# cvg/nice-slam

Hardware: NVIDIA H100
Metric: rendered rays/sec (higher is better)
Workload: dtype f32

## Files before the change

nice_slam_b200/csrc/nsb_aux.cu:

```cuda
#include <cstdarg>
#include <cstdio>
#include <cstring>
#include <cuda_fp16.h>
#include "nsb_common.cuh"
#include "nsb_seeds.cuh"
#include "nsb_geom.cuh"

namespace nsb {

static thread_local char g_err[512] = "";
void set_error(const char* fmt, ...) {
  va_list ap; va_start(ap, fmt); vsnprintf(g_err, sizeof(g_err), fmt, ap); va_end(ap);
}
int check_cuda(cudaError_t e, const char* what) {
  if (e == cudaSuccess) return NSB_OK;
  set_error("%s: %s", what, cudaGetErrorString(e));
  (void)cudaGetLastError();
  return NSB_ERR_CUDA;
}

struct PackArgs { nsb_decoder_params p[4]; float* packed[4]; float* flat[4]; int present[4]; };
__device__ __forceinline__ bool pk_mine(int& e) { return (e++ % (int)gridDim.y) == (int)blockIdx.y; }
constexpr int kPackSlices = 32;

// ... 175 lines not shown
  __shared__ float red[32];
  float m = -INFINITY;
  for (int i = threadIdx.x; i < n; i += blockDim.x) m = fmaxf(m, gt[i]);
  for (int o = 16; o > 0; o >>= 1) m = fmaxf(m, __shfl_xor_sync(0xffffffffu, m, o));
  if ((threadIdx.x & 31) == 0) red[threadIdx.x >> 5] = m;
  __syncthreads();
  if (threadIdx.x < 32) {
    m = threadIdx.x < (blockDim.x >> 5) ? red[threadIdx.x] : -INFINITY;
    for (int o = 16; o > 0; o >>= 1) m = fmaxf(m, __shfl_xor_sync(0xffffffffu, m, o));
    if (threadIdx.x == 0) {
      if (n <= 0) m = 0.0f;
      out2[0] = m;
      out2[1] = __fmul_rn(m, 1.2f);
    }
  }
  if (px.world > 1) {
    __shared__ uint32_t s_seq;
    __syncthreads();
    const uint32_t seq = peer_begin(px, 0, &s_seq);
    const int par = seq & 1u;
    if ((int)threadIdx.x < px.world) ll_put_f32(px.peer[threadIdx.x] + kXMaxOff + ((size_t)par * NSB_MAX_PEERS + px.rank) * 16, out2[0], seq);
    if (threadIdx.x < 32) {
      float mm = -INFINITY;
      if ((int)threadIdx.x < px.world) mm = ll_get_f32(px.peer[px.rank] + kXMaxOff + ((size_t)par * NSB_MAX_PEERS + threadIdx.x) * 16, seq, px, 0);
      for (int o = 16; o > 0; o >>= 1) mm = fmaxf(mm, __shfl_xor_sync(0xffffffffu, mm, o));
      if (threadIdx.x == 0) { out2[0] = mm; out2[1] = __fmul_rn(mm, 1.2f); }
    }
    peer_end(px, 0, seq);
  }
}

struct Bound6 { double b[6]; };
__global__ void prefilter_kernel(const float* __restrict__ ro, const float* __restrict__ rd, const float* __restrict__ gt,
                                 int n, const Bound6 B, uint8_t* __restrict__ keep) {
  const int i = blockIdx.x * blockDim.x + threadIdx.x;
  if (i >= n) return;
  const float o[3] = {ro[3 * i], ro[3 * i + 1], ro[3 * i + 2]}, d[3] = {rd[3 * i], rd[3 * i + 1], rd[3 * i + 2]};
  const double t = ray_far_bb(B.b, o, d);
  keep[i] = (t >= (double)gt[i]) ? 1 : 0;
}

__global__ void tracking_seeds_kernel(const double* __restrict__ depth, const double* __restrict__ var, const float* __restrict__ rgb,
                                      const float* __restrict__ gt, const double* __restrict__ gt_rgb, int n, double w_color,
                                      int handle_dynamic, int use_color, const double* __restrict__ pool, int n_pool,
                                      double* __restrict__ g_depth, float* __restrict__ g_rgb,
                                      double* __restrict__ loss, double* __restrict__ res, const PeerX px) {
  __shared__ __align__(16) unsigned char scratch[kSeedsScratchBytes];
// ... 720 lines not shown
```

nice_slam_b200/csrc/nsb_seeds.cuh:

```cuda
#pragma once
#include <cstdio>
#include "nsb_common.cuh"

namespace nsb {

constexpr long long kPeerWaitCycles = 20000000000ll;
constexpr size_t kXMaxOff = 0, kXSumOff = 256, kXSumStride = 256, kXPoolOff = kXSumOff + 2 * NSB_MAX_PEERS * kXSumStride;
__host__ __device__ inline size_t peer_pool_plain_off(int max_n) { return kXPoolOff + (size_t)2 * NSB_MAX_PEERS * (size_t)max_n * 16; }
__host__ __device__ inline size_t peer_buffer_bytes(int max_n) { return peer_pool_plain_off(max_n) + (size_t)NSB_MAX_PEERS * (size_t)max_n * sizeof(double); }
__device__ __forceinline__ void ll_put(unsigned char* slot16, double v, uint32_t seq) {
  const unsigned long long b = (unsigned long long)__double_as_longlong(v);
  const unsigned long long w0 = ((unsigned long long)seq << 32) | (b & 0xffffffffull), w1 = ((unsigned long long)seq << 32) | (b >> 32);
  asm volatile("st.relaxed.sys.global.v2.u64 [%0], {%1, %2};" ::"l"(slot16), "l"(w0), "l"(w1) : "memory");
}
__device__ __forceinline__ double ll_get(const unsigned char* slot16, uint32_t seq, const PeerX& px, int c) {
  unsigned long long w0, w1;
  const long long t0 = clock64();
  for (;;) {
    asm volatile("ld.relaxed.sys.global.v2.u64 {%0, %1}, [%2];" : "=l"(w0), "=l"(w1) : "l"(slot16) : "memory");
    if ((uint32_t)(w0 >> 32) == seq && (uint32_t)(w1 >> 32) == seq) break;
    if (clock64() - t0 > kPeerWaitCycles) { printf("nsb: peer exchange timed out (rank %d, channel %d, seq %u)\n", px.rank, c, seq); __trap(); }
  }
  return __longlong_as_double((long long)((w1 << 32) | (w0 & 0xffffffffull)));
}
__device__ __forceinline__ void ll_put_f32(unsigned char* slot8, float v, uint32_t seq) {
  const unsigned long long w = ((unsigned long long)seq << 32) | (unsigned long long)__float_as_uint(v);
  asm volatile("st.relaxed.sys.global.u64 [%0], %1;" ::"l"(slot8), "l"(w) : "memory");
}
__device__ __forceinline__ float ll_get_f32(const unsigned char* slot8, uint32_t seq, const PeerX& px, int c) {
  unsigned long long w;
  const long long t0 = clock64();
  for (;;) {
    asm volatile("ld.relaxed.sys.global.u64 %0, [%1];" : "=l"(w) : "l"(slot8) : "memory");
    if ((uint32_t)(w >> 32) == seq) break;
    if (clock64() - t0 > kPeerWaitCycles) { printf("nsb: peer exchange timed out (rank %d, channel %d, seq %u)\n", px.rank, c, seq); __trap(); }
  }
  return __uint_as_float((uint32_t)w);
}
__device__ __forceinline__ void peer_end(const PeerX& px, int c, uint32_t seq) {
  __syncthreads();
  if (threadIdx.x == 0) px.counter[c] = (unsigned long long)seq;
}
__device__ __forceinline__ uint32_t peer_begin(const PeerX& px, int c, uint32_t* s_seq) {
  if (threadIdx.x == 0) *s_seq = (uint32_t)(px.counter[c] + 1ull);
  __syncthreads();
  return *s_seq;
}

__device__ __forceinline__ float peer_max_all_ctas(const PeerX& px, float local, uint32_t* s_seq) {
  if (threadIdx.x == 0) *s_seq = (uint32_t)(px.counter[0] + 1ull);
  __syncthreads();
  const uint32_t seq = *s_seq;
  const int par = seq & 1u;
  __syncthreads();
  if (blockIdx.x == 0 && (int)threadIdx.x < px.world)
    ll_put_f32(px.peer[threadIdx.x] + kXMaxOff + ((size_t)par * NSB_MAX_PEERS + px.rank) * 16, local, seq);
  float m = -INFINITY;
  if (threadIdx.x < 32) {
    if ((int)threadIdx.x < px.world) m = ll_get_f32(px.peer[px.rank] + kXMaxOff + ((size_t)par * NSB_MAX_PEERS + threadIdx.x) * 16, seq, px, 0);
    for (int o = 16; o > 0; o >>= 1) m = fmaxf(m, __shfl_xor_sync(0xffffffffu, m, o));
    if (threadIdx.x == 0) *reinterpret_cast<float*>(s_seq) = m;
  }
  __syncthreads();
  m = *reinterpret_cast<const float*>(s_seq);
  __syncthreads();
  return m;
}
__device__ __forceinline__ void peer_advance(const PeerX& px, int c) {
  px.counter[c] = px.counter[c] + 1ull;
}
__device__ __forceinline__ void peer_sum13(const PeerX& px, const double* tot, int n_val, double* out, uint32_t* s_seq) {
  const uint32_t seq = peer_begin(px, 2, s_seq);
  const int par = seq & 1u;
  for (int i = threadIdx.x; i < n_val * px.world; i += blockDim.x) {
    const int r = i / n_val, k = i - n_val * r;
    ll_put(px.peer[r] + kXSumOff + ((size_t)par * NSB_MAX_PEERS + px.rank) * kXSumStride + (size_t)k * 16, tot[k], seq);
  }
  if ((int)threadIdx.x < n_val) {
    double v = 0.0;
    for (int r = 0; r < px.world; r++) v += ll_get(px.peer[px.rank] + kXSumOff + ((size_t)par * NSB_MAX_PEERS + r) * kXSumStride + (size_t)threadIdx.x * 16, seq, px, 2);
    out[threadIdx.x] = v;
  }
  peer_end(px, 2, seq);
}

constexpr int kMedianDirect = 512;
constexpr int kSeedsScratchBytes = 34 * 8 + kMedianDirect * 8 + (256 + 8 + 2 + 2) * 4;

__device__ __forceinline__ double block_sum(double v, double* red) {
  for (int o = 16; o > 0; o >>= 1) v += __shfl_xor_sync(0xffffffffu, v, o);
  if ((threadIdx.x & 31) == 0) red[threadIdx.x >> 5] = v;
  __syncthreads();
  double t = 0.0;
  if (threadIdx.x < 32) {
    t = threadIdx.x < (blockDim.x >> 5) ? red[threadIdx.x] : 0.0;
    for (int o = 16; o > 0; o >>= 1) t += __shfl_xor_sync(0xffffffffu, t, o);
  }
  __syncthreads();
  return t;
}
__device__ __forceinline__ double sgn(double x) { return (x > 0.0) - (x < 0.0); }

__device__ __forceinline__ void tracking_seeds_body(const double* depth, const double* var, const float* rgb,
// ... 6 lines not shown
  unsigned long long& med_key = *reinterpret_cast<unsigned long long*>(red + 33);
  unsigned long long* keys = reinterpret_cast<unsigned long long*>(red + 34);
  int* hist = reinterpret_cast<int*>(keys + kMedianDirect);
  int* wtot = hist + 256;
  int* sel = wtot + 8;
  uint32_t* s_seq_p = reinterpret_cast<uint32_t*>(sel + 2);
  for (int i = threadIdx.x; i < n; i += blockDim.x)
    res[i] = fabs((double)gt[i] - depth[i]) / sqrt(var[i] + 1e-10);
  __syncthreads();
  if (handle_dynamic) {
    const double* mp = pool != nullptr ? pool : res;
    int np = pool != nullptr ? n_pool : n;
    int pool_pitch = 0;
    if (px.world > 1) {
      const uint32_t seq = peer_begin(px, 1, s_seq_p);
      const int par = seq & 1u;
      for (int i = threadIdx.x; i < n * px.world; i += blockDim.x) {
        const int r = i / n, j = i - r * n;
        ll_put(px.peer[r] + kXPoolOff + (((size_t)par * NSB_MAX_PEERS + px.rank) * px.max_n + j) * 16, res[j], seq);
      }
      double* plain = reinterpret_cast<double*>(px.peer[px.rank] + peer_pool_plain_off(px.max_n));
      for (int i = threadIdx.x; i < n * px.world; i += blockDim.x) {
        const int r = i / n, j = i - r * n;
        plain[(size_t)r * px.max_n + j] = ll_get(px.peer[px.rank] + kXPoolOff + (((size_t)par * NSB_MAX_PEERS + r) * px.max_n + j) * 16, seq, px, 1);
      }
      peer_end(px, 1, seq);
      mp = plain;
      np = n * px.world; pool_pitch = px.max_n;
    }
    auto pool_at = [&](int i) { return pool_pitch ? mp[(size_t)(i / n) * pool_pitch + (i % n)] : mp[i]; };
    const int k = (np - 1) / 2;
    auto select_direct = [&](int cnt, int want) {
      if (cnt > 256) {
        int m = 512;
        for (int i = cnt + threadIdx.x; i < m; i += blockDim.x) keys[i] = ~0ull;
        __syncthreads();
        for (int k2 = 2; k2 <= m; k2 <<= 1)
          for (int j = k2 >> 1; j > 0; j >>= 1) {
            for (int t = threadIdx.x; t < m / 2; t += blockDim.x) {
              const int i = ((t & ~(j - 1)) << 1) | (t & (j - 1));
              const unsigned long long x = keys[i], y = keys[i | j];
              if ((x > y) == ((i & k2) == 0)) { keys[i] = y; keys[i | j] = x; }
            }
            __syncthreads();
          }
        if (threadIdx.x == 0) med_key = keys[want];
        __syncthreads();
// ... 123 lines not shown
```

nice_slam_b200/csrc/nsb_tc.cuh:

```cuda
#pragma once

namespace nsb {
namespace tc {

#ifdef NSB_PHASE_TIMING
__device__ long long g_phase[64];
__device__ long long g_phase_last;
#define NSB_PH(id) do { if (blockIdx.x == 0 && threadIdx.x == 0) { const long long c_ = clock64(); ::nsb::tc::g_phase[id] += c_ - ::nsb::tc::g_phase_last; ::nsb::tc::g_phase_last = c_; } } while (0)
#define NSB_PH_RESET() do { if (blockIdx.x == 0 && threadIdx.x == 0) ::nsb::tc::g_phase_last = clock64(); } while (0)
#else
#define NSB_PH(id) do { } while (0)
#define NSB_PH_RESET() do { } while (0)
#endif

constexpr int TM = 128;
constexpr int kThreads = 512;
constexpr int kCG = kThreads / TM;
constexpr int kCW = 32 / kCG;
constexpr int kKQ = kCW / 4;

__device__ __forceinline__ float to_tf32(float x) { return __uint_as_float(__float_as_uint(x) & 0xffffe000u); }

__device__ __forceinline__ int canon_q(int r, int kq, int K) { return ((r >> 3) * (K >> 2) + kq) * 32 + (r & 7) * 4; }

// ... 3 lines not shown
  h.x = to_tf32(v.x); h.y = to_tf32(v.y); h.z = to_tf32(v.z); h.w = to_tf32(v.w);
  l.x = v.x - h.x; l.y = v.y - h.y; l.z = v.z - h.z; l.w = v.w - h.w;
  *reinterpret_cast<float4*>(hi + idx) = h;
  *reinterpret_cast<float4*>(lo + idx) = l;
}

__device__ __forceinline__ uint64_t make_desc(const float* smem, uint32_t lbo_bytes, uint32_t sbo_bytes) {
  uint64_t d = 0;
  d |= (uint64_t)((smem_u32(smem) >> 4) & 0x3FFF);
  d |= (uint64_t)((lbo_bytes >> 4) & 0x3FFF) << 16;
  d |= (uint64_t)((sbo_bytes >> 4) & 0x3FFF) << 32;
  return d;
}

constexpr int kAccCols = 256;
constexpr int kAccSlotsPerSm = 4;
constexpr int kAccMaxSm = 144;
__device__ float g_acc_pool[(size_t)kAccMaxSm * kAccSlotsPerSm * kAccCols * TM];
__device__ int g_acc_lock[kAccMaxSm * kAccSlotsPerSm];
__shared__ float* s_acc;
__device__ __forceinline__ uint32_t acc_acquire() {
  uint32_t smid;
  asm volatile("mov.u32 %0, %%smid;" : "=r"(smid));
  if (smid >= (uint32_t)kAccMaxSm) { printf("nsb: SM id %u beyond the accumulator pool\n", smid); __trap(); }
  const long long t0 = clock64();
  for (;;) {
    for (int k = 0; k < kAccSlotsPerSm; k++) {
      const int s = (int)smid * kAccSlotsPerSm + k;
      if (atomicCAS(&g_acc_lock[s], 0, 1) == 0) {
        __threadfence();
        s_acc = g_acc_pool + (size_t)s * kAccCols * TM;
        return (uint32_t)s;
      }
    }
    if (clock64() - t0 > 4000000000ll) { printf("nsb: no free accumulator slot on SM %u\n", smid); __trap(); }
  }
}
__device__ __forceinline__ void acc_release(uint32_t slot) { __threadfence(); atomicExch(&g_acc_lock[slot], 0); }
__device__ __forceinline__ const float* acc_col(uint32_t taddr) { return s_acc + (size_t)(taddr & 0xffffu) * TM + (taddr >> 16) + (threadIdx.x & 31); }

__device__ __forceinline__ void wg_fence() { asm volatile("wgmma.fence.sync.aligned;" ::: "memory"); }
__device__ __forceinline__ void wg_commit_wait() {
  asm volatile("wgmma.commit_group.sync.aligned;" ::: "memory");
  asm volatile("wgmma.wait_group.sync.aligned 0;" ::: "memory");
}
__device__ __forceinline__ void wg_commit() { asm volatile("wgmma.commit_group.sync.aligned;" ::: "memory"); }
__device__ __forceinline__ void wg_wait0() { asm volatile("wgmma.wait_group.sync.aligned 0;" ::: "memory"); }
__device__ __forceinline__ void fence_acc(float (&d)[16]) {
#pragma unroll
  for (int e = 0; e < 16; e++) asm volatile("" : "+f"(d[e])::"memory");
}
#define NSB_WG_D16 "+f"(d[0]), "+f"(d[1]), "+f"(d[2]), "+f"(d[3]), "+f"(d[4]), "+f"(d[5]), "+f"(d[6]), "+f"(d[7]), \
                   "+f"(d[8]), "+f"(d[9]), "+f"(d[10]), "+f"(d[11]), "+f"(d[12]), "+f"(d[13]), "+f"(d[14]), "+f"(d[15])
__device__ __forceinline__ void wgmma_tf32_n32(float (&d)[16], uint64_t da, uint64_t db) {
  asm volatile("{\n\t.reg .pred p;\n\tsetp.ne.b32 p, 1, 0;\n\t"
               "wgmma.mma_async.sync.aligned.m64n32k8.f32.tf32.tf32 "
               "{%0,%1,%2,%3,%4,%5,%6,%7,%8,%9,%10,%11,%12,%13,%14,%15}, %16, %17, p, 1, 1;\n\t}"
               : NSB_WG_D16 : "l"(da), "l"(db));
// ... 457 lines not shown
```

nice_slam_b200/csrc/nsb_tile.cuh:

```cuda
#pragma once

namespace nsb {
namespace tl {

using tc::TM;
constexpr int kThreads = 256;
constexpr int kEpiThreads = kThreads;
constexpr int kCG = 2, kCW = 16, kKQ = 4;
constexpr int kSlots = 4;
constexpr int kSlotFloatsFwd = 2560;
constexpr int kSlotFloatsBwd = 2048;
constexpr int kABufFloats = 2 * TM * 32;
constexpr int kMaxTileRays = 18;
constexpr int kMinSamples = 8;
constexpr long long kWaitCycles = 4000000000ll;

enum { B_FULL = 0, B_EMPTY = 4, B_HDR = 8, B_AREADY = 10, B_DONE = 12, kNumBars = 14 };

__device__ __forceinline__ bool mbar_try(uint64_t* bar, uint32_t parity) {
  uint32_t ok;
  asm volatile("{\n\t.reg .pred p;\n\tmbarrier.try_wait.parity.shared::cta.b64 p, [%1], %2;\n\tselp.b32 %0, 1, 0, p;\n\t}"
               : "=r"(ok) : "r"(smem_u32(bar)), "r"(parity) : "memory");
  return ok != 0;
}
__device__ __forceinline__ bool mbar_test(uint64_t* bar, uint32_t parity) {
  uint32_t ok;
  asm volatile("{\n\t.reg .pred p;\n\tmbarrier.test_wait.parity.shared::cta.b64 p, [%1], %2;\n\tselp.b32 %0, 1, 0, p;\n\t}"
               : "=r"(ok) : "r"(smem_u32(bar)), "r"(parity) : "memory");
  return ok != 0;
}
__device__ __forceinline__ void mbar_wait_b(uint64_t* bar, uint32_t parity) {
  if (mbar_try(bar, parity)) return;
  const long long t0 = clock64();
  while (!mbar_try(bar, parity)) {
    if (clock64() - t0 > kWaitCycles) { printf("nsb: mbarrier wait timed out (block %d thread %d bar %p parity %u)\n", blockIdx.x, threadIdx.x, (void*)bar, parity); __trap(); }
  }
}
__device__ __forceinline__ void mbar_arrive(uint64_t* bar) {
  asm volatile("mbarrier.arrive.shared::cta.b64 _, [%0];" ::"r"(smem_u32(bar)) : "memory");
}
__device__ __forceinline__ void epi_sync() { __syncthreads(); }

struct TileSmem {
  float* a[2];
  float* ring;
  int slot_floats;
  float* hdr;
  uint64_t* bars;
  uint32_t* tmem;
  unsigned char* extra;
};
__host__ __device__ constexpr size_t common_bytes(bool bwd) {
  return (2 * (size_t)kABufFloats + (size_t)kSlots * (bwd ? kSlotFloatsBwd : kSlotFloatsFwd) + 2 * kHdrFloats) * 4 + 128;
}
__device__ __forceinline__ void carve(unsigned char* base, TileSmem& t, bool bwd) {
  float* f = reinterpret_cast<float*>(base);
  t.a[0] = f; f += kABufFloats; t.a[1] = f; f += kABufFloats;
  t.slot_floats = bwd ? kSlotFloatsBwd : kSlotFloatsFwd;
// ... 46 lines not shown
}
__device__ __forceinline__ void loader_top_up(Loader& L, const TileSmem& t, uint32_t issued) {
  while (!loader_done(L) && L.loaded < issued + kSlots) {
    if (L.loaded >= kSlots) { const uint32_t prev = L.loaded - kSlots; if (!mbar_test(t.bars + B_EMPTY + (prev & (kSlots - 1)), (prev >> 2) & 1u)) return; }
    loader_issue(L, t);
  }
}
__device__ __forceinline__ void load_header(const KParams& P, const TileSmem& t, int lv, int hb) {
  uint64_t* bar = t.bars + B_HDR + hb;
  mbar_expect_tx(bar, kHdrFloats * 4u);
  tma_bulk_g2s(t.hdr + hb * kHdrFloats, P.in.packed[lv] + op_fwd_offset(lv), kHdrFloats * 4u, bar);
}

struct Issuer {
  Loader L;
  uint32_t issued;
  uint32_t g;
};
__device__ __forceinline__ void issuer_wait_operands(Issuer& I, const TileSmem& t, int b, uint32_t parity) {
  uint64_t* bar = t.bars + B_AREADY + b;
  const long long t0 = clock64();
  while (!mbar_test(bar, parity)) {
    if (threadIdx.x == 0) loader_top_up(I.L, t, I.issued);
    if (clock64() - t0 > kWaitCycles) { printf("nsb: issuer timed out waiting for operands (block %d)\n", blockIdx.x); __trap(); }
  }
}
__device__ __forceinline__ const float* issuer_unit(Issuer& I, const TileSmem& t, uint32_t k = 0) {
  if (threadIdx.x == 0) {
    loader_top_up(I.L, t, I.issued);
    while (I.L.loaded <= I.issued + k) loader_refill(I.L, t, I.issued);
  }
  const uint32_t u = I.issued + k;
  const int slot = u & (kSlots - 1);
  mbar_wait_b(t.bars + B_FULL + slot, (u >> 2) & 1u);
  return t.ring + slot * t.slot_floats;
}
__device__ __forceinline__ const float* issued_unit(const Issuer& I, const TileSmem& t, uint32_t k) { return t.ring + ((I.issued + k) & (kSlots - 1)) * t.slot_floats; }

__device__ __forceinline__ uint32_t cvt_h2(float lo_elem, float hi_elem) {
  uint32_t r;
  asm("cvt.rn.satfinite.f16x2.f32 %0, %1, %2;" : "=r"(r) : "f"(hi_elem), "f"(lo_elem));
  return r;
}
__device__ __forceinline__ void split_h2(float x, float y, uint32_t& h, uint32_t& l) {
  h = cvt_h2(x, y);
  const float2 f = __half22float2(*reinterpret_cast<const __half2*>(&h));
  l = cvt_h2(x - f.x, y - f.y);
}
__device__ __forceinline__ void put4_h(float* tile, int r, int kq, const float4 v) {
  unsigned char* hi = reinterpret_cast<unsigned char*>(tile) + (((r >> 3) * 4 + (kq >> 1)) * 128 + (r & 7) * 16 + (kq & 1) * 8);
  uint2 h, l;
  split_h2(v.x, v.y, h.x, l.x); split_h2(v.z, v.w, h.y, l.y);
  *reinterpret_cast<uint2*>(hi) = h;
  *reinterpret_cast<uint2*>(hi + TM * 32 * 2) = l;
}
__device__ __forceinline__ void put16_h(float* tile, int r, int cg, const float (&v)[kCW]) {
#pragma unroll
  for (int c = 0; c < 2; c++) {
    unsigned char* hi = reinterpret_cast<unsigned char*>(tile) + (((r >> 3) * 4 + 2 * cg + c) * 128 + (r & 7) * 16);
    uint4 h, l;
    split_h2(v[8 * c], v[8 * c + 1], h.x, l.x); split_h2(v[8 * c + 2], v[8 * c + 3], h.y, l.y);
    split_h2(v[8 * c + 4], v[8 * c + 5], h.z, l.z); split_h2(v[8 * c + 6], v[8 * c + 7], h.w, l.w);
    *reinterpret_cast<uint4*>(hi) = h;
    *reinterpret_cast<uint4*>(hi + TM * 32 * 2) = l;
  }
}
template <bool H16>
__device__ __forceinline__ void mma_rows(float (&d)[16], const float* a, int ka0, const float* b, int N, int KB, int c, int ksteps) {
  const uint32_t g = (threadIdx.x >> 7) & 1u;
  const int esz = H16 ? 2 : 4, kcm = H16 ? 8 : 4;
  const uint32_t sbo_a = (32u / kcm) * 128u, sbo_b = (uint32_t)(KB / kcm) * 128u;
  uint64_t ah = tc::make_desc(a + (ka0 / kcm) * 32, 128u, sbo_a), bh = tc::make_desc(b, 128u, sbo_b);
  ah += (uint64_t)((8u * sbo_a * g) >> 4);
  bh += (uint64_t)((4u * sbo_b * (uint32_t)c) >> 4);
  const uint64_t al = ah + (uint64_t)((TM * 32 * esz) >> 4), bl = bh + (uint64_t)((N * KB * esz) >> 4);
#pragma unroll 1
  for (int ks = 0; ks < ksteps; ks++) {
    const uint64_t o = 16u * (uint64_t)ks;
    if (H16) { tc::wgmma_f16_n32(d, al + o, bh + o); tc::wgmma_f16_n32(d, ah + o, bl + o); tc::wgmma_f16_n32(d, ah + o, bh + o); }
    else { tc::wgmma_tf32_n32(d, al + o, bh + o); tc::wgmma_tf32_n32(d, ah + o, bl + o); tc::wgmma_tf32_n32(d, ah + o, bh + o); }
  }
}
__device__ __forceinline__ void release_units(Issuer& I, const TileSmem& t, uint32_t count, uint64_t* done = nullptr) {
  if ((threadIdx.x & 127) == 0) {
    for (uint32_t k = 0; k < count; k++) mbar_arrive(t.bars + B_EMPTY + ((I.issued + k) & (kSlots - 1)));
    if (done != nullptr) mbar_arrive(done);
  }
  I.issued += count;
}
__device__ __forceinline__ void wg_bar_sync() {
  if (threadIdx.x >> 7) asm volatile("bar.sync 2, 128;" ::: "memory");
  else asm volatile("bar.sync 1, 128;" ::: "memory");
}
__device__ __forceinline__ void zero16(float (&d)[16]) {
#pragma unroll
  for (int e = 0; e < 16; e++) d[e] = 0.0f;
}
__device__ __forceinline__ void put2(float* hi, int r, int c, float a, float b) {
  float* hp = hi + tc::canon_q(r, c >> 2, 32) + (c & 3);
  const float h0 = tc::to_tf32(a), h1 = tc::to_tf32(b);
  *reinterpret_cast<float2*>(hp) = make_float2(h0, h1);
  *reinterpret_cast<float2*>(hp + TM * 32) = make_float2(a - h0, b - h1);
}

__device__ __forceinline__ void publish(const TileSmem& t, int b) {
  fence_proxy_async();
  __syncwarp();
  if ((threadIdx.x & 31) == 0) mbar_arrive(t.bars + B_AREADY + b);
}
__device__ __forceinline__ void wait_group(const TileSmem& t, uint32_t m) {
  mbar_wait_b(t.bars + B_DONE + (m & 1u), (m >> 1) & 1u);
}

struct GatherPass {
  float4 v[8];
  float w[8];
  int src_lane;
};
template <bool FAST>
// ... 72 lines not shown
__device__ __forceinline__ float4* d2_frag(int i) { return reinterpret_cast<float4*>(tc::s_acc + ((size_t)i * kThreads + threadIdx.x) * 16); }
__device__ __forceinline__ void ld_frag(const float4* p, float (&d)[16]) {
#pragma unroll
  for (int k = 0; k < 4; k++) { const float4 v = p[k]; d[4 * k] = v.x; d[4 * k + 1] = v.y; d[4 * k + 2] = v.z; d[4 * k + 3] = v.w; }
}
__device__ __forceinline__ void st_frag(float4* p, const float (&d)[16]) {
#pragma unroll
  for (int k = 0; k < 4; k++) p[k] = make_float4(d[4 * k], d[4 * k + 1], d[4 * k + 2], d[4 * k + 3]);
}
template <bool H16 = false>
__device__ __forceinline__ void issue_fc(Issuer& I, const TileSmem& t, int half) {
  constexpr int nu = H16 ? 2 : 4;
  const int b = I.g & 1;
  issuer_wait_operands(I, t, b, (I.g >> 1) & 1u);
#pragma unroll 1
  for (int u = 0; u < nu; u++) issuer_unit(I, t, u);
#pragma unroll 1
  for (int c = 0; c < 5; c++) {
    float4* p = d2_frag(c);
    float d[16];
    if (half == 0) zero16(d); else ld_frag(p, d);
    tc::wg_fence();
#pragma unroll
    for (int u = 0; u < nu; u++) mma_rows<H16>(d, t.a[b], H16 ? 16 * u : 8 * u, issued_unit(I, t, u), 160, H16 ? 16 : 8, c, 1);
    tc::wg_commit(); tc::wg_wait0(); tc::fence_acc(d);
    st_frag(p, d);
  }
  release_units(I, t, nu, t.bars + B_DONE + b);
  I.g++;
}
template <bool H16 = false>
__device__ __forceinline__ void issue_l0(Issuer& I, const TileSmem& t, float (&d1)[16], float (&d3)[16]) {
  constexpr int nu = H16 ? 1 : 2;
  const int b = I.g & 1;
  issuer_wait_operands(I, t, b, (I.g >> 1) & 1u);
#pragma unroll 1
  for (int u = 0; u < nu; u++) issuer_unit(I, t, u);
  tc::wg_fence();
#pragma unroll
  for (int u = 0; u < nu; u++) {
    mma_rows<H16>(d1, t.a[b], 16 * u, issued_unit(I, t, u), 64, H16 ? 32 : 16, 0, 2);
    mma_rows<H16>(d3, t.a[b], 16 * u, issued_unit(I, t, u), 64, H16 ? 32 : 16, 1, 2);
  }
  tc::wg_commit(); tc::wg_wait0(); tc::fence_acc(d1); tc::fence_acc(d3);
  release_units(I, t, nu, t.bars + B_DONE + b);
  I.g++;
}
template <bool H16 = false>
__device__ __forceinline__ void issue_h(Issuer& I, const TileSmem& t, float (&d1)[16], const float (&d3)[16], const float* hbuf, int i) {
  const float* w = issuer_unit(I, t);
  if (i == 3) {
#pragma unroll
    for (int e = 0; e < 16; e++) d1[e] = d3[e];
  } else {
    zero16(d1);
  }
  tc::wg_fence();
  mma_rows<H16>(d1, hbuf, 0, w, 32, 32, 0, H16 ? 2 : 4);
  tc::wg_commit();
}

template <bool H16 = false>
__device__ __forceinline__ void epi_forward(const KParams& P, const TileSmem& t, Issuer& I, int lv, const PointGeom& G, uint32_t& n, int hb, uint32_t hdr_parity,
                                            float (&out)[4], uint32_t* __restrict__ masks, float* __restrict__ acts, int npts) {
  const int row = threadIdx.x & (TM - 1), cg = threadIdx.x >> 7, warp = threadIdx.x >> 5, lane = threadIdx.x & 31;
  const bool xyz = lv != 0;
  const int cd = op_cd(lv), no = lv == 3 ? 4 : 1;
  const float* hdr = t.hdr + hb * kHdrFloats;
  float d1[16], d3[16];
  zero16(d1); zero16(d3);
  if (xyz) {
    for (int half = 0; half < cd / 32; half++) {
      if (n >= 2) wait_group(t, n - 2);
      if (threadIdx.x == 0) loader_top_up(I.L, t, I.issued);
      gather_tile<H16>(P.in.grid[half == 0 ? lv : 1], t.a[n & 1], G.xn, warp, lane);
      NSB_PH(1);
      publish(t, n & 1); n++;
      issue_fc<H16>(I, t, half);
      NSB_PH(2);
    }
    mbar_wait_b(t.bars + B_HDR + hb, hdr_parity);
    for (int blk = 0; blk < 3; blk++) {
      if (n >= 2) wait_group(t, n - 2);
      if (threadIdx.x == 0) loader_top_up(I.L, t, I.issued);
      NSB_PH(6);
      embed_tile<H16>(t.a[n & 1], hdr + 464, G.pf, row, cg, blk);
      NSB_PH(3);
      publish(t, n & 1); n++;
      issue_l0<H16>(I, t, d1, d3);
      NSB_PH(4);
    }
  } else {
    if (n >= 2) wait_group(t, n - 2);
    gather_tile<H16>(P.in.grid[0], t.a[n & 1], G.xnc, warp, lane);
    publish(t, n & 1); n++;
    issue_l0<H16>(I, t, d1, d3);
    mbar_wait_b(t.bars + B_HDR + hb, hdr_parity);
  }
  st_frag(d2_frag(5), d3);
  float* hbuf = t.a[n & 1];
  const int wg = threadIdx.x >> 7, q = lane & 3;
  const int r0 = 64 * wg + 16 * (warp & 3) + (lane >> 2);
#pragma unroll 1
  for (int i = 0; i < 5; i++) {
    float v2[16];
    if (xyz) ld_frag(d2_frag(i), v2);
    if (i > 0) { tc::wg_wait0(); tc::fence_acc(d1); release_units(I, t, 1); }
    if (threadIdx.x == 0) loader_top_up(I.L, t, I.issued);
    NSB_PH(7);
    uint32_t m0 = 0, m1 = 0;
#pragma unroll
    for (int e = 0; e < 16; e++) {
      const int c = 8 * (e >> 2) + 2 * q + (e & 1);
      const float u = d1[e] + hdr[i * 32 + c];
      const uint32_t bit = u > 0.0f ? 1u << (8 * (e >> 2) + (e & 1)) : 0u;
      if (e & 2) m1 |= bit; else m0 |= bit;
      float h = u > 0.0f ? u : 0.0f;
      if (xyz) h += v2[e] + hdr[160 + i * 32 + c];
      d1[e] = h;
    }
    if (masks != nullptr) {
      m0 <<= 2 * q; m1 <<= 2 * q;
      m0 |= __shfl_xor_sync(0xffffffffu, m0, 1); m1 |= __shfl_xor_sync(0xffffffffu, m1, 1);
      m0 |= __shfl_xor_sync(0xffffffffu, m0, 2); m1 |= __shfl_xor_sync(0xffffffffu, m1, 2);
      if (q == 0 && r0 < npts) masks[(size_t)r0 * 15 + i] = m0;
      if (q == 1 && r0 + 8 < npts) masks[(size_t)(r0 + 8) * 15 + i] = m1;
    }
    if (acts != nullptr) {
#pragma unroll
      for (int e = 0; e < 16; e += 2) {
// ... 1 lines not shown
        if (r < npts) __stcg(reinterpret_cast<float2*>(acts + (size_t)r * 160 + i * 32 + c), make_float2(d1[e], d1[e + 1]));
      }
    }
    if (i == 4) break;
    if (i == 2) ld_frag(d2_frag(5), d3);
#pragma unroll
    for (int e = 0; e < 16; e += 2) {
      const int r = r0 + 8 * ((e >> 1) & 1), c = 8 * (e >> 2) + 2 * q;
      if (H16) {
        unsigned char* hp = reinterpret_cast<unsigned char*>(hbuf) + (((r >> 3) * 4 + (c >> 3)) * 128 + (r & 7) * 16 + (c & 7) * 2);
        uint32_t hh, ll;
        split_h2(d1[e], d1[e + 1], hh, ll);
        *reinterpret_cast<uint32_t*>(hp) = hh;
        *reinterpret_cast<uint32_t*>(hp + TM * 32 * 2) = ll;
      } else {
        put2(hbuf, r, c, d1[e], d1[e + 1]);
      }
    }
    NSB_PH(8);
    fence_proxy_async();
    wg_bar_sync();
    issue_h<H16>(I, t, d1, d3, hbuf, i + 1);
    NSB_PH(9);
  }
  NSB_PH(8);
  float s0[4], s1[4];
#pragma unroll
  for (int o = 0; o < 4; o++) {
    s0[o] = s1[o] = 0.0f;
    if (o < no) {
#pragma unroll
      for (int e = 0; e < 16; e++) {
        const float w = hdr[336 + o * 32 + 8 * (e >> 2) + 2 * q + (e & 1)];
        if (e & 2) s1[o] = fmaf(d1[e], w, s1[o]); else s0[o] = fmaf(d1[e], w, s0[o]);
      }
    }
    s0[o] += __shfl_xor_sync(0xffffffffu, s0[o], 1); s1[o] += __shfl_xor_sync(0xffffffffu, s1[o], 1);
    s0[o] += __shfl_xor_sync(0xffffffffu, s0[o], 2); s1[o] += __shfl_xor_sync(0xffffffffu, s1[o], 2);
  }
  constexpr int kWgHiFloats = 64 * 32 / (H16 ? 2 : 1);
  auto part = [&](int r) { return reinterpret_cast<float4*>(hbuf + (r >> 6) * kWgHiFloats + (r & 63) * 4); };
  if (q == 0) *part(r0) = make_float4(s0[0], s0[1], s0[2], s0[3]);
  if (q == 1) *part(r0 + 8) = make_float4(s1[0], s1[1], s1[2], s1[3]);
  epi_sync();
  {
    const float4 v = *part(row);
// ... 32 lines not shown
__device__ __forceinline__ void gather_tile_kt(const nsb_grid& g, float* c_hi, int lo_off, const float xn[3], int warp, int lane) {
  const bool fast = grid_fast(g);
  const int qd = warp & 3, it0 = (warp >> 2) * 4, q = lane & 7;
#pragma unroll 1
  for (int it = it0; it < it0 + 4; it++) {
    GatherPass A;
    if (fast) gather_issue<true>(g, xn, it, lane, A); else gather_issue<false>(g, xn, it, lane, A);
    float4 acc = make_float4(0.f, 0.f, 0.f, 0.f);
#pragma unroll
    for (int k = 0; k < 8; k++) {
      const float w = A.w[k];
      acc.x = fmaf(A.v[k].x, w, acc.x); acc.y = fmaf(A.v[k].y, w, acc.y); acc.z = fmaf(A.v[k].z, w, acc.z); acc.w = fmaf(A.v[k].w, w, acc.w);
    }
    const int p = qd * 32 + A.src_lane;
    float4 xh, xl; split4(acc, xh, xl);
    const float hv[4] = {xh.x, xh.y, xh.z, xh.w}, lv[4] = {xl.x, xl.y, xl.z, xl.w};
#pragma unroll
    for (int c = 0; c < 4; c++) { const int o = kt_idx(4 * q + c, p); c_hi[o] = hv[c]; c_hi[lo_off + o] = lv[c]; }
  }
}
__device__ __forceinline__ void wg_group(WgSmem& w, int part, float* dst, int pitch, int n_rows, bool transposed3 = false) {
  fence_proxy_async();
  __syncthreads();
  if (threadIdx.x < 128) {
    const uint64_t ah = tc::make_desc(w.du, 128u, 4096u), al = ah + (uint64_t)((kWgALo * 4) >> 4);
    const uint64_t bh = tc::make_desc(w.b, 128u, 4096u), bl = bh + (uint64_t)((kWgBLo * 4) >> 4);
    float d[16];
#pragma unroll
    for (int e = 0; e < 16; e++) d[e] = 0.0f;
    tc::wg_fence();
#pragma unroll 1
    for (int ks = 0; ks < TM / 8; ks++) {
      const uint64_t o = 16u * (uint64_t)ks;
      tc::wgmma_tf32_n32(d, al + o, bh + o); tc::wgmma_tf32_n32(d, ah + o, bl + o); tc::wgmma_tf32_n32(d, ah + o, bh + o);
    }
    tc::wg_commit_wait();
    if ((threadIdx.x >> 6) == part) {
#pragma unroll
      for (int e = 0; e < 16; e += 2) {
        int r, c; tc::frag_rc(e, r, c); r -= 32 * part;
        if (r >= n_rows) continue;
        if (transposed3) {
          if (c < 3) atomicAdd(dst + (size_t)c * pitch + r, d[e]);
          if (c + 1 < 3) atomicAdd(dst + (size_t)(c + 1) * pitch + r, d[e + 1]);
        } else {
          red_add_v2(dst + (size_t)r * pitch + c, d[e], d[e + 1]);
        }
      }
    }
  }
  __syncthreads();
}
__device__ __forceinline__ float warp_colsum16(const float (&v)[kCW], int lane) {
  float a[8];
// ... 23 lines not shown
  for (int j = 0; j < 2; j++) { const float give = (lane & 8) ? b[j] : b[j + 2], keep = (lane & 8) ? b[j + 2] : b[j]; c[j] = keep + __shfl_xor_sync(0xffffffffu, give, 8); }
  const float give = (lane & 4) ? c[0] : c[1], keep = (lane & 4) ? c[1] : c[0];
  return keep + __shfl_xor_sync(0xffffffffu, give, 4);
}
__device__ __forceinline__ int frag_colsum_col(int lane) {
  const int j = ((lane >> 4) & 1) * 4 + ((lane >> 3) & 1) * 2 + ((lane >> 2) & 1);
  return 8 * (j >> 1) + 2 * (lane & 3) + (j & 1);
}

struct BwdExtra {
  double dp[TM * 3];
  double z[TM];
  float gocc[TM];
  float wgt[TM];
  float gc[kMaxTileRays * 3];
};
__device__ __forceinline__ void bwd_gout(const BwdExtra& X, int lv, int r, int npts, int off0, int S, float (&go)[4]) {
  go[0] = go[1] = go[2] = go[3] = 0.0f;
  if (r >= npts) return;
  if (lv == 3) { const float w = X.wgt[r]; const float* gc = X.gc + 3 * ((off0 + r) / S); go[0] = w * gc[0]; go[1] = w * gc[1]; go[2] = w * gc[2]; }
  else go[0] = X.gocc[r];
}

__device__ __forceinline__ void issue_bwd_layer(Issuer& I, const TileSmem& t, int lv, int i, float (&d1)[16], float (&dc)[16], float (&fa)[16]) {
  const bool xyz = lv != 0;
  const int ndc = xyz ? op_cd(lv) / 32 : 0, nd1 = i >= 1 ? 1 : 0, ndf = (i == 3 || i == 0) ? op_firstp(lv) / 32 : 0;
  const int fmax = i == 0 ? 2 : 1;
  int f0 = 0;
  int nf = min(ndf, fmax);
  int nu = ndc + nd1 + nf;
#pragma unroll 1
  for (int wave = 0; nu > 0; wave++) {
    if (nf > 0) { if (i == 0) ld_frag(d2_frag(f0), fa); else zero16(fa); }
    if (nf > 1) ld_frag(d2_frag(f0 + 1), d1);
    if (wave == 0) {
      if (xyz && i == 4) zero16(dc);
      if (nd1) zero16(d1);
    }
#pragma unroll 1
    for (int u = 0; u < nu; u++) issuer_unit(I, t, u);
    const int k = wave == 0 ? ndc + nd1 : 0;
    tc::wg_fence();
    if (wave == 0) {
      if (xyz) mma_rows<false>(dc, t.a[0], 0, issued_unit(I, t, 0), 32, 32, 0, 4);
      if (nd1) mma_rows<false>(d1, t.a[1], 0, issued_unit(I, t, ndc), 32, 32, 0, 4);
    }
    if (nf > 0) mma_rows<false>(fa, t.a[1], 0, issued_unit(I, t, k), 32, 32, 0, 4);
    if (nf > 1) mma_rows<false>(d1, t.a[1], 0, issued_unit(I, t, k + 1), 32, 32, 0, 4);
    tc::wg_commit(); tc::wg_wait0();
    tc::fence_acc(dc); tc::fence_acc(d1); tc::fence_acc(fa);
    if (nf > 0) st_frag(d2_frag(f0), fa);
    if (nf > 1) st_frag(d2_frag(f0 + 1), d1);
    release_units(I, t, nu);
    f0 += nf;
    nf = min(ndf - f0, fmax);
    nu = nf;
  }
}

__device__ __forceinline__ int bwd_dpe_off(int r) { return (r >> 6) * (64 * 32) + (r & 63) * 4; }
template <bool WG>
__device__ __forceinline__ void epi_backward(const KParams& P, const TileSmem& t, Issuer& I, const BwdExtra& X, int lv, const PointGeom& G, int hb, uint32_t hdr_parity,
                                             const uint32_t* __restrict__ masks, int npts, int off0, long long gp0, WgSmem* w = nullptr, const float* acts_row = nullptr) {
  const int row = threadIdx.x & (TM - 1), cg = threadIdx.x >> 7, warp = threadIdx.x >> 5;
  const int lane = threadIdx.x & 31, q = lane & 3;
  const int r0 = 64 * (threadIdx.x >> 7) + 16 * (warp & 3) + (lane >> 2);
  const int S = P.S;
  using DW = Dec<3>;
  float creg[kCW];
  const bool xyz = lv != 0;
  const float* hdr = t.hdr + hb * kHdrFloats;
  uint32_t m01 = 0, m23 = 0, m4 = 0;
  {
    const uint32_t* w0 = masks + (size_t)(r0 < npts ? r0 : npts - 1) * 15;
    const uint32_t* w1 = masks + (size_t)(r0 + 8 < npts ? r0 + 8 : npts - 1) * 15;
#pragma unroll
    for (int i = 0; i < 5; i++) {
      const uint32_t v = ((w0[i] >> (2 * q)) & 0x03030303u) | (((w1[i] >> (2 * q)) & 0x03030303u) << 2);
      if (i == 4) m4 = v; else if (i & 2) m23 |= v << (4 * (i & 1)); else m01 |= v << (4 * (i & 1));
    }
// ... 632 lines not shown
```

Before: 1.065 million.

## Strip device printf, template MMA k-steps, and restructure wgmma issue loops

Removes printf calls from the timeout and trap paths so their argument-marshalling code and stack usage drop out of hot kernels. Makes the MMA k-step count a template parameter so the wgmma loops fully unroll. Templates the backward layer issue on the configuration, and adds opaque zeroing of accumulators. Also moves the forward-loop wait/release and the next fragment load to after the next issue, so the MMAs overlap more work. The trade-offs are lost diagnostic messages on traps, and possible register-pressure or code-size growth from the extra unrolling and templating.

```diff
diff --git a/nice_slam_b200/csrc/nsb_aux.cu b/nice_slam_b200/csrc/nsb_aux.cu
--- a/nice_slam_b200/csrc/nsb_aux.cu
+++ b/nice_slam_b200/csrc/nsb_aux.cu
@@ -221,7 +221,7 @@
     if ((int)threadIdx.x < px.world) ll_put_f32(px.peer[threadIdx.x] + kXMaxOff + ((size_t)par * NSB_MAX_PEERS + px.rank) * 16, out2[0], seq);
     if (threadIdx.x < 32) {
       float mm = -INFINITY;
-      if ((int)threadIdx.x < px.world) mm = ll_get_f32(px.peer[px.rank] + kXMaxOff + ((size_t)par * NSB_MAX_PEERS + threadIdx.x) * 16, seq, px, 0);
+      if ((int)threadIdx.x < px.world) mm = ll_get_f32(px.peer[px.rank] + kXMaxOff + ((size_t)par * NSB_MAX_PEERS + threadIdx.x) * 16, seq);
       for (int o = 16; o > 0; o >>= 1) mm = fmaxf(mm, __shfl_xor_sync(0xffffffffu, mm, o));
       if (threadIdx.x == 0) { out2[0] = mm; out2[1] = __fmul_rn(mm, 1.2f); }
     }
diff --git a/nice_slam_b200/csrc/nsb_seeds.cuh b/nice_slam_b200/csrc/nsb_seeds.cuh
--- a/nice_slam_b200/csrc/nsb_seeds.cuh
+++ b/nice_slam_b200/csrc/nsb_seeds.cuh
@@ -13,13 +13,13 @@
   const unsigned long long w0 = ((unsigned long long)seq << 32) | (b & 0xffffffffull), w1 = ((unsigned long long)seq << 32) | (b >> 32);
   asm volatile("st.relaxed.sys.global.v2.u64 [%0], {%1, %2};" ::"l"(slot16), "l"(w0), "l"(w1) : "memory");
 }
-__device__ __forceinline__ double ll_get(const unsigned char* slot16, uint32_t seq, const PeerX& px, int c) {
+__device__ __forceinline__ double ll_get(const unsigned char* slot16, uint32_t seq) {
   unsigned long long w0, w1;
   const long long t0 = clock64();
   for (;;) {
     asm volatile("ld.relaxed.sys.global.v2.u64 {%0, %1}, [%2];" : "=l"(w0), "=l"(w1) : "l"(slot16) : "memory");
     if ((uint32_t)(w0 >> 32) == seq && (uint32_t)(w1 >> 32) == seq) break;
-    if (clock64() - t0 > kPeerWaitCycles) { printf("nsb: peer exchange timed out (rank %d, channel %d, seq %u)\n", px.rank, c, seq); __trap(); }
+    if (clock64() - t0 > kPeerWaitCycles) __trap();
   }
   return __longlong_as_double((long long)((w1 << 32) | (w0 & 0xffffffffull)));
 }
@@ -27,13 +27,13 @@
   const unsigned long long w = ((unsigned long long)seq << 32) | (unsigned long long)__float_as_uint(v);
   asm volatile("st.relaxed.sys.global.u64 [%0], %1;" ::"l"(slot8), "l"(w) : "memory");
 }
-__device__ __forceinline__ float ll_get_f32(const unsigned char* slot8, uint32_t seq, const PeerX& px, int c) {
+__device__ __forceinline__ float ll_get_f32(const unsigned char* slot8, uint32_t seq) {
   unsigned long long w;
   const long long t0 = clock64();
   for (;;) {
     asm volatile("ld.relaxed.sys.global.u64 %0, [%1];" : "=l"(w) : "l"(slot8) : "memory");
     if ((uint32_t)(w >> 32) == seq) break;
-    if (clock64() - t0 > kPeerWaitCycles) { printf("nsb: peer exchange timed out (rank %d, channel %d, seq %u)\n", px.rank, c, seq); __trap(); }
+    if (clock64() - t0 > kPeerWaitCycles) __trap();
   }
   return __uint_as_float((uint32_t)w);
 }
@@ -57,7 +57,7 @@
     ll_put_f32(px.peer[threadIdx.x] + kXMaxOff + ((size_t)par * NSB_MAX_PEERS + px.rank) * 16, local, seq);
   float m = -INFINITY;
   if (threadIdx.x < 32) {
-    if ((int)threadIdx.x < px.world) m = ll_get_f32(px.peer[px.rank] + kXMaxOff + ((size_t)par * NSB_MAX_PEERS + threadIdx.x) * 16, seq, px, 0);
+    if ((int)threadIdx.x < px.world) m = ll_get_f32(px.peer[px.rank] + kXMaxOff + ((size_t)par * NSB_MAX_PEERS + threadIdx.x) * 16, seq);
     for (int o = 16; o > 0; o >>= 1) m = fmaxf(m, __shfl_xor_sync(0xffffffffu, m, o));
     if (threadIdx.x == 0) *reinterpret_cast<float*>(s_seq) = m;
   }
@@ -78,7 +78,7 @@
   }
   if ((int)threadIdx.x < n_val) {
     double v = 0.0;
-    for (int r = 0; r < px.world; r++) v += ll_get(px.peer[px.rank] + kXSumOff + ((size_t)par * NSB_MAX_PEERS + r) * kXSumStride + (size_t)threadIdx.x * 16, seq, px, 2);
+    for (int r = 0; r < px.world; r++) v += ll_get(px.peer[px.rank] + kXSumOff + ((size_t)par * NSB_MAX_PEERS + r) * kXSumStride + (size_t)threadIdx.x * 16, seq);
     out[threadIdx.x] = v;
   }
   peer_end(px, 2, seq);
@@ -131,7 +131,7 @@
       double* plain = reinterpret_cast<double*>(px.peer[px.rank] + peer_pool_plain_off(px.max_n));
       for (int i = threadIdx.x; i < n * px.world; i += blockDim.x) {
         const int r = i / n, j = i - r * n;
-        plain[(size_t)r * px.max_n + j] = ll_get(px.peer[px.rank] + kXPoolOff + (((size_t)par * NSB_MAX_PEERS + r) * px.max_n + j) * 16, seq, px, 1);
+        plain[(size_t)r * px.max_n + j] = ll_get(px.peer[px.rank] + kXPoolOff + (((size_t)par * NSB_MAX_PEERS + r) * px.max_n + j) * 16, seq);
       }
       peer_end(px, 1, seq);
       mp = plain;
diff --git a/nice_slam_b200/csrc/nsb_tc.cuh b/nice_slam_b200/csrc/nsb_tc.cuh
--- a/nice_slam_b200/csrc/nsb_tc.cuh
+++ b/nice_slam_b200/csrc/nsb_tc.cuh
@@ -49,7 +49,7 @@
 __device__ __forceinline__ uint32_t acc_acquire() {
   uint32_t smid;
   asm volatile("mov.u32 %0, %%smid;" : "=r"(smid));
-  if (smid >= (uint32_t)kAccMaxSm) { printf("nsb: SM id %u beyond the accumulator pool\n", smid); __trap(); }
+  if (smid >= (uint32_t)kAccMaxSm) __trap();
   const long long t0 = clock64();
   for (;;) {
     for (int k = 0; k < kAccSlotsPerSm; k++) {
@@ -60,7 +60,7 @@
         return (uint32_t)s;
       }
     }
-    if (clock64() - t0 > 4000000000ll) { printf("nsb: no free accumulator slot on SM %u\n", smid); __trap(); }
+    if (clock64() - t0 > 4000000000ll) __trap();
   }
 }
 __device__ __forceinline__ void acc_release(uint32_t slot) { __threadfence(); atomicExch(&g_acc_lock[slot], 0); }
diff --git a/nice_slam_b200/csrc/nsb_tile.cuh b/nice_slam_b200/csrc/nsb_tile.cuh
--- a/nice_slam_b200/csrc/nsb_tile.cuh
+++ b/nice_slam_b200/csrc/nsb_tile.cuh
@@ -33,7 +33,7 @@
   if (mbar_try(bar, parity)) return;
   const long long t0 = clock64();
   while (!mbar_try(bar, parity)) {
-    if (clock64() - t0 > kWaitCycles) { printf("nsb: mbarrier wait timed out (block %d thread %d bar %p parity %u)\n", blockIdx.x, threadIdx.x, (void*)bar, parity); __trap(); }
+    if (clock64() - t0 > kWaitCycles) __trap();
   }
 }
 __device__ __forceinline__ void mbar_arrive(uint64_t* bar) {
@@ -126,7 +126,7 @@
   const long long t0 = clock64();
   while (!mbar_test(bar, parity)) {
     if (threadIdx.x == 0) loader_top_up(I.L, t, I.issued);
-    if (clock64() - t0 > kWaitCycles) { printf("nsb: issuer timed out waiting for operands (block %d)\n", blockIdx.x); __trap(); }
+    if (clock64() - t0 > kWaitCycles) __trap();
   }
 }
 __device__ __forceinline__ const float* issuer_unit(Issuer& I, const TileSmem& t, uint32_t k = 0) {
@@ -169,8 +169,8 @@
     *reinterpret_cast<uint4*>(hi + TM * 32 * 2) = l;
   }
 }
-template <bool H16>
-__device__ __forceinline__ void mma_rows(float (&d)[16], const float* a, int ka0, const float* b, int N, int KB, int c, int ksteps) {
+template <bool H16, int ksteps>
+__device__ __forceinline__ void mma_rows(float (&d)[16], const float* a, int ka0, const float* b, int N, int KB, int c) {
   const uint32_t g = (threadIdx.x >> 7) & 1u;
   const int esz = H16 ? 2 : 4, kcm = H16 ? 8 : 4;
   const uint32_t sbo_a = (32u / kcm) * 128u, sbo_b = (uint32_t)(KB / kcm) * 128u;
@@ -178,7 +178,7 @@
   ah += (uint64_t)((8u * sbo_a * g) >> 4);
   bh += (uint64_t)((4u * sbo_b * (uint32_t)c) >> 4);
   const uint64_t al = ah + (uint64_t)((TM * 32 * esz) >> 4), bl = bh + (uint64_t)((N * KB * esz) >> 4);
-#pragma unroll 1
+#pragma unroll
   for (int ks = 0; ks < ksteps; ks++) {
     const uint64_t o = 16u * (uint64_t)ks;
     if (H16) { tc::wgmma_f16_n32(d, al + o, bh + o); tc::wgmma_f16_n32(d, ah + o, bl + o); tc::wgmma_f16_n32(d, ah + o, bh + o); }
@@ -199,6 +199,10 @@
 __device__ __forceinline__ void zero16(float (&d)[16]) {
 #pragma unroll
   for (int e = 0; e < 16; e++) d[e] = 0.0f;
+}
+__device__ __forceinline__ void zero16_opaque(float (&d)[16]) {
+#pragma unroll
+  for (int e = 0; e < 16; e++) asm volatile("mov.b32 %0, 0;" : "=f"(d[e])::"memory");
 }
 __device__ __forceinline__ void put2(float* hi, int r, int c, float a, float b) {
   float* hp = hi + tc::canon_q(r, c >> 2, 32) + (c & 3);
@@ -317,7 +321,7 @@
     if (half == 0) zero16(d); else ld_frag(p, d);
     tc::wg_fence();
 #pragma unroll
-    for (int u = 0; u < nu; u++) mma_rows<H16>(d, t.a[b], H16 ? 16 * u : 8 * u, issued_unit(I, t, u), 160, H16 ? 16 : 8, c, 1);
+    for (int u = 0; u < nu; u++) mma_rows<H16, 1>(d, t.a[b], H16 ? 16 * u : 8 * u, issued_unit(I, t, u), 160, H16 ? 16 : 8, c);
     tc::wg_commit(); tc::wg_wait0(); tc::fence_acc(d);
     st_frag(p, d);
   }
@@ -334,8 +338,8 @@
   tc::wg_fence();
 #pragma unroll
   for (int u = 0; u < nu; u++) {
-    mma_rows<H16>(d1, t.a[b], 16 * u, issued_unit(I, t, u), 64, H16 ? 32 : 16, 0, 2);
-    mma_rows<H16>(d3, t.a[b], 16 * u, issued_unit(I, t, u), 64, H16 ? 32 : 16, 1, 2);
+    mma_rows<H16, 2>(d1, t.a[b], 16 * u, issued_unit(I, t, u), 64, H16 ? 32 : 16, 0);
+    mma_rows<H16, 2>(d3, t.a[b], 16 * u, issued_unit(I, t, u), 64, H16 ? 32 : 16, 1);
   }
   tc::wg_commit(); tc::wg_wait0(); tc::fence_acc(d1); tc::fence_acc(d3);
   release_units(I, t, nu, t.bars + B_DONE + b);
@@ -351,7 +355,7 @@
     zero16(d1);
   }
   tc::wg_fence();
-  mma_rows<H16>(d1, hbuf, 0, w, 32, 32, 0, H16 ? 2 : 4);
+  mma_rows<H16, H16 ? 2 : 4>(d1, hbuf, 0, w, 32, 32, 0);
   tc::wg_commit();
 }
 
@@ -389,6 +393,7 @@
     if (n >= 2) wait_group(t, n - 2);
     gather_tile<H16>(P.in.grid[0], t.a[n & 1], G.xnc, warp, lane);
     publish(t, n & 1); n++;
+    zero16_opaque(d1); zero16_opaque(d3);
     issue_l0<H16>(I, t, d1, d3);
     mbar_wait_b(t.bars + B_HDR + hb, hdr_parity);
   }
@@ -396,11 +401,10 @@
   float* hbuf = t.a[n & 1];
   const int wg = threadIdx.x >> 7, q = lane & 3;
   const int r0 = 64 * wg + 16 * (warp & 3) + (lane >> 2);
+  float v2[16];
+  if (xyz) ld_frag(d2_frag(0), v2);
 #pragma unroll 1
   for (int i = 0; i < 5; i++) {
-    float v2[16];
-    if (xyz) ld_frag(d2_frag(i), v2);
-    if (i > 0) { tc::wg_wait0(); tc::fence_acc(d1); release_units(I, t, 1); }
     if (threadIdx.x == 0) loader_top_up(I.L, t, I.issued);
     NSB_PH(7);
     uint32_t m0 = 0, m1 = 0;
@@ -448,6 +452,8 @@
     wg_bar_sync();
     issue_h<H16>(I, t, d1, d3, hbuf, i + 1);
     NSB_PH(9);
+    if (xyz) ld_frag(d2_frag(i + 1), v2);
+    tc::wg_wait0(); tc::fence_acc(d1); release_units(I, t, 1);
   }
   NSB_PH(8);
   float s0[4], s1[4];
@@ -526,14 +532,13 @@
 __device__ __forceinline__ void wg_group(WgSmem& w, int part, float* dst, int pitch, int n_rows, bool transposed3 = false) {
   fence_proxy_async();
   __syncthreads();
-  if (threadIdx.x < 128) {
+  if (__shfl_sync(0xffffffffu, threadIdx.x >> 7, 0) == 0) {
     const uint64_t ah = tc::make_desc(w.du, 128u, 4096u), al = ah + (uint64_t)((kWgALo * 4) >> 4);
     const uint64_t bh = tc::make_desc(w.b, 128u, 4096u), bl = bh + (uint64_t)((kWgBLo * 4) >> 4);
     float d[16];
-#pragma unroll
-    for (int e = 0; e < 16; e++) d[e] = 0.0f;
+    zero16_opaque(d);
     tc::wg_fence();
-#pragma unroll 1
+#pragma unroll
     for (int ks = 0; ks < TM / 8; ks++) {
       const uint64_t o = 16u * (uint64_t)ks;
       tc::wgmma_tf32_n32(d, al + o, bh + o); tc::wgmma_tf32_n32(d, ah + o, bl + o); tc::wgmma_tf32_n32(d, ah + o, bh + o);
@@ -603,40 +608,46 @@
   else go[0] = X.gocc[r];
 }
 
-__device__ __forceinline__ void issue_bwd_layer(Issuer& I, const TileSmem& t, int lv, int i, float (&d1)[16], float (&dc)[16], float (&fa)[16]) {
-  const bool xyz = lv != 0;
-  const int ndc = xyz ? op_cd(lv) / 32 : 0, nd1 = i >= 1 ? 1 : 0, ndf = (i == 3 || i == 0) ? op_firstp(lv) / 32 : 0;
-  const int fmax = i == 0 ? 2 : 1;
-  int f0 = 0;
-  int nf = min(ndf, fmax);
-  int nu = ndc + nd1 + nf;
-#pragma unroll 1
-  for (int wave = 0; nu > 0; wave++) {
-    if (nf > 0) { if (i == 0) ld_frag(d2_frag(f0), fa); else zero16(fa); }
-    if (nf > 1) ld_frag(d2_frag(f0 + 1), d1);
-    if (wave == 0) {
-      if (xyz && i == 4) zero16(dc);
-      if (nd1) zero16(d1);
-    }
+template <bool DC, int NDF, bool L0>
+__device__ __forceinline__ void issue_bwd_layer_t(Issuer& I, const TileSmem& t, int ndc, float (&d1)[16], float (&dc)[16], float (&fa)[16]) {
+  constexpr int ND1 = L0 ? 0 : 1, FMAX = L0 ? 2 : 1;
+  constexpr int kWaves = NDF > FMAX ? (NDF + FMAX - 1) / FMAX : 1;
+#pragma unroll
+  for (int wave = 0; wave < kWaves; wave++) {
+    const int f0 = wave * FMAX;
+    const int nf = NDF - f0 < FMAX ? NDF - f0 : FMAX;
+    const int k = wave == 0 ? ndc + ND1 : 0;
+    const int nu = k + nf;
 #pragma unroll 1
     for (int u = 0; u < nu; u++) issuer_unit(I, t, u);
-    const int k = wave == 0 ? ndc + nd1 : 0;
+    if (nf > 0) { if (L0) ld_frag(d2_frag(f0), fa); else zero16_opaque(fa); }
+    if (nf > 1) ld_frag(d2_frag(f0 + 1), d1);
+    if (wave == 0 && ND1) zero16_opaque(d1);
     tc::wg_fence();
     if (wave == 0) {
-      if (xyz) mma_rows<false>(dc, t.a[0], 0, issued_unit(I, t, 0), 32, 32, 0, 4);
-      if (nd1) mma_rows<false>(d1, t.a[1], 0, issued_unit(I, t, ndc), 32, 32, 0, 4);
-    }
-    if (nf > 0) mma_rows<false>(fa, t.a[1], 0, issued_unit(I, t, k), 32, 32, 0, 4);
-    if (nf > 1) mma_rows<false>(d1, t.a[1], 0, issued_unit(I, t, k + 1), 32, 32, 0, 4);
+      if (DC) mma_rows<false, 4>(dc, t.a[0], 0, issued_unit(I, t, 0), 32, 32, 0);
+      if (ND1) mma_rows<false, 4>(d1, t.a[1], 0, issued_unit(I, t, ndc), 32, 32, 0);
+    }
+    if (nf > 0) mma_rows<false, 4>(fa, t.a[1], 0, issued_unit(I, t, k), 32, 32, 0);
+    if (nf > 1) mma_rows<false, 4>(d1, t.a[1], 0, issued_unit(I, t, k + 1), 32, 32, 0);
     tc::wg_commit(); tc::wg_wait0();
     tc::fence_acc(dc); tc::fence_acc(d1); tc::fence_acc(fa);
     if (nf > 0) st_frag(d2_frag(f0), fa);
     if (nf > 1) st_frag(d2_frag(f0 + 1), d1);
     release_units(I, t, nu);
-    f0 += nf;
-    nf = min(ndf - f0, fmax);
-    nu = nf;
-  }
+  }
+}
+template <bool XYZ>
+__device__ __forceinline__ void issue_bwd_layer_x(Issuer& I, const TileSmem& t, int ndc, int i, float (&d1)[16], float (&dc)[16], float (&fa)[16]) {
+  constexpr int NDF = op_firstp(XYZ ? 1 : 0) / 32;
+  if (XYZ && i == 4) zero16_opaque(dc);
+  if (i == 3) issue_bwd_layer_t<XYZ, NDF, false>(I, t, ndc, d1, dc, fa);
+  else if (i == 0) issue_bwd_layer_t<XYZ, NDF, true>(I, t, ndc, d1, dc, fa);
+  else issue_bwd_layer_t<XYZ, 0, false>(I, t, ndc, d1, dc, fa);
+}
+__device__ __forceinline__ void issue_bwd_layer(Issuer& I, const TileSmem& t, int lv, int i, float (&d1)[16], float (&dc)[16], float (&fa)[16]) {
+  if (lv != 0) issue_bwd_layer_x<true>(I, t, op_cd(lv) / 32, i, d1, dc, fa);
+  else issue_bwd_layer_x<false>(I, t, 0, i, d1, dc, fa);
 }
 
 __device__ __forceinline__ int bwd_dpe_off(int r) { return (r >> 6) * (64 * 32) + (r & 63) * 4; }
```

Result: faster. 1.203 million, median of 6 (+13.0%).
